# Gaurav14cs17/Bayer_Low_light_Image_Enhancement

Measured on AMD Instinct MI355X. Metric: megapixels/sec RawFormer-S 512x512 RAW->sRGB, higher is better.
Workload: dtype f32; 1 GPU; RawFormer-S(FLCA) dim=32, batch=8 of packed 4x512x512 synthetic Bayer per GPU; frames_per_gpu=8, variant=flca, weights=synthetic (seeded, random-init scale), parallelism=batch-sharded x1, device=AMD Radeon Graphics

## Files before the change

### bayer_low_light_image_enhancement_amd/csrc/rf_conv3x3.hip

```cpp
#include <cstdio>
#include <cstdlib>
#include "rf_common.h"

namespace rf {

static constexpr int KC = 8;
static constexpr int kKsCounters = 4096;
typedef unsigned u32x4 __attribute__((ext_vector_type(4)));

template <int NCO, int LOG2_RW, int RPW, int NWV, bool KS = false>
__global__ void __launch_bounds__(64 * NWV, (NWV >= 8 || NCO >= 3) ? 1 : 2) conv3x3_kernel(Conv3x3Args a, int ngroups, int tiles_x, int ntiles, int vec) {
    constexpr int NTHR = 64 * NWV;
    constexpr int TAPS = 18;
    constexpr int NM = 6;
    constexpr int RW = 1 << LOG2_RW;
    constexpr int TW = 64 / RW;
    constexpr int TH = NWV * RW * RPW;
    static_assert(RPW == 1 || RW == 1, "two row groups per wave only with one row per group");
    constexpr int RS = TW + 8;
    constexpr int PS = ((TH + 2) * RS + 63) / 64 * 64;
    constexpr int NIN = KC * (TH + 2) * (TW + 2);
    constexpr int EPT = (NIN + NTHR - 1) / NTHR;
    constexpr int NW4 = 2 * TAPS * NCO * 16;
    constexpr int WPT = (NW4 + NTHR - 1) / NTHR;
    constexpr int BUF = KC * PS + 2 * TAPS * NCO * 64;
    __shared__ __attribute__((aligned(16))) float lds[2 * BUF];
    __shared__ float bias_l[NCO * 16];

    const int tid = threadIdx.x;
    const int lane = tid & 63, wave = tid >> 6;
    const int j = lane & 15, kq = lane >> 4;
    const int rowj = j / (16 / RW), cg = j % (16 / RW);
    const int grp = blockIdx.x % ngroups;
    const int wg = blockIdx.x / ngroups;
    const int b = blockIdx.y;
    const int h = a.h, w = a.w;
    const int NT = (a.Cout + 15) >> 4;
    const int t0 = grp * NCO;
    const int nchunks_all = (a.Cin + KC - 1) / KC;
    const int ksplit = KS ? (int)gridDim.z : 1, kz = KS ? (int)blockIdx.z : 0;
    const int ch_lo = KS ? (int)((long)kz * nchunks_all / ksplit) : 0, ch_hi = KS ? (int)((long)(kz + 1) * nchunks_all / ksplit) : nchunks_all;
    const float* xb = a.x + (size_t)b * a.x_bstride;
    const size_t chunk_stride = a.unshuffle_in ? (size_t)(KC / 4) * 4 * h * w : (size_t)KC * h * w;

    constexpr unsigned OOB = 0x80000000u;
    int prc[EPT];
    short loff[EPT];
    static_assert(PS - (TH + 2) * RS >= 16, "plane padding holds the dummy slots");
    const int dummy = (tid & 7) * PS + (TH + 2) * RS + ((tid >> 3) & 15);
#pragma unroll
    for (int i = 0; i < EPT; ++i) {
        const int idx = tid + NTHR * i;
        const int c = idx % (TW + 2);
        const int r = (idx / (TW + 2)) % (TH + 2);
        const int cl = idx / ((TW + 2) * (TH + 2));
        prc[i] = idx < NIN ? (cl << 16) | (r << 8) | c : -1;
        loff[i] = (short)(idx < NIN ? cl * PS + r * RS + c : dummy);
    }
    unsigned wvoff[WPT];
#pragma unroll
    for (int i = 0; i < WPT; ++i) {
        const int idx = tid + NTHR * i;
        const int l4 = idx % 16;
        const int t = (idx / 16) % NCO;
        const int kt = idx / (16 * NCO);
        const bool ok = idx < NW4 && t0 + t < NT;
        wvoff[i] = ok ? (unsigned)(((kt * NT + t0 + t) * 64 + l4 * 4) * 4) : OOB;
    }
    const int w_chunk_bytes = 2 * TAPS * NT * 64 * 4;
    const size_t plane_bytes = (size_t)h * w * 4;

    unsigned voff[EPT];
    int x0 = 0, y0 = 0;
    auto plan_tile = [&](int tile) {
        const int tx = tile % tiles_x, ty = tile / tiles_x;
        x0 = tx * TW;
        y0 = ty * TH;
#pragma unroll
        for (int i = 0; i < EPT; ++i) {
            int e = prc[i];
            asm volatile("" : "+v"(e));
            const int cl = e >> 16;
            const int y = y0 - 1 + ((e >> 8) & 255), x = x0 - 1 + (e & 255);
            const bool ok = e >= 0 && (unsigned)y < (unsigned)h && (unsigned)x < (unsigned)w;
            const int off_m = ((cl >> 2) * 2 * h + 2 * y + ((cl >> 1) & 1)) * (2 * w) + 2 * x + (cl & 1);
            const int off_p = (cl * h + y) * w + x;
            voff[i] = ok ? (unsigned)(4 * (a.unshuffle_in ? off_m : off_p)) : OOB;
        }
    };
    float xin[EPT];
    float4 win[WPT];
    auto load_chunk = [&](int ch) {
        const int cl_lim = min(KC, a.Cin - ch * KC);
        const float* src = xb + (size_t)ch * chunk_stride;
        const __amdgpu_buffer_rsrc_t rx = __builtin_amdgcn_make_buffer_rsrc(
            const_cast<float*>(src), 0, (int)(a.unshuffle_in ? (size_t)(cl_lim / 4) * 4 * plane_bytes : (size_t)cl_lim * plane_bytes), 0x00020000);
        const __amdgpu_buffer_rsrc_t rw = __builtin_amdgcn_make_buffer_rsrc(
            const_cast<float*>(a.wp) + (size_t)ch * (w_chunk_bytes / 4), 0, w_chunk_bytes, 0x00020000);
#pragma unroll
        for (int i = 0; i < EPT; ++i) xin[i] = __uint_as_float(__builtin_amdgcn_raw_buffer_load_b32(rx, (int)voff[i], 0, 0));
#pragma unroll
        for (int i = 0; i < WPT; ++i) {
            const u32x4 v = __builtin_amdgcn_raw_buffer_load_b128(rw, (int)wvoff[i], 0, 0);
            win[i] = make_float4(__uint_as_float(v.x), __uint_as_float(v.y), __uint_as_float(v.z), __uint_as_float(v.w));
        }
    };
    auto store_chunk = [&](int buf) {
        float* li = lds + buf * BUF;
        float* lw = li + KC * PS;
#pragma unroll
        for (int i = 0; i < EPT; ++i) {
            float v = xin[i];
            if (a.clamp_in) v = fminf(fmaxf(v, 0.f), 1.f);
            li[loff[i]] = v;
        }
#pragma unroll
        for (int i = 0; i < WPT; ++i) {
            const int idx = tid + NTHR * i;
            if (idx < NW4) *reinterpret_cast<float4*>(lw + idx * 4) = win[i];
        }
    };

    f32x4 acc[RPW][NCO][NM];

    const int nwg = gridDim.x / ngroups;
    int tile = wg;
    const int tile_end = ntiles;
    if (tile >= tile_end) return;
    if (tid < NCO * 16) {
        const int co = 16 * t0 + tid;
        bias_l[tid] = (a.bias && co < a.Cout) ? a.bias[co] : 0.f;
    }
    plan_tile(tile);
    load_chunk(ch_lo);
    store_chunk(0);
    __syncthreads();
    int buf = 0;
    float* outb = a.out + (size_t)b * a.out_bstride;
    for (; tile < tile_end; tile += nwg) {
        const int ex0 = x0, ey0 = y0;
#pragma unroll
        for (int rr = 0; rr < RPW; ++rr)
#pragma unroll
            for (int t = 0; t < NCO; ++t)
#pragma unroll
                for (int g = 0; g < NM; ++g) acc[rr][t][g] = (f32x4){0.f, 0.f, 0.f, 0.f};
        for (int ch = ch_lo; ch < ch_hi; ++ch) {
            const bool last = ch + 1 == ch_hi;
            const bool more = !last || tile + nwg < tile_end;
            const int nch = last ? ch_lo : ch + 1;
            if (last && more) plan_tile(tile + nwg);
            if (more) load_chunk(nch);
            const float* lds_in = lds + buf * BUF;
            const float* lds_w = lds_in + KC * PS;
            const int nks = (a.Cin - ch * KC > 4) ? 2 : 1;
#pragma unroll
            for (int ks = 0; ks < 2; ++ks) {
                if (ks >= nks) break;
                const float* lp = lds_in + (ks * 4 + kq) * PS + (wave * RW * RPW + rowj) * RS + 4 * cg;
#pragma unroll
                for (int ir = 0; ir < RPW + 2; ++ir) {
                    const float4 lo = *reinterpret_cast<const float4*>(lp + ir * RS);
                    const float4 hi = *reinterpret_cast<const float4*>(lp + ir * RS + 4);
                    float d[NM];
                    {
                        const float p = fmaf(-4.f, lo.z, hi.x), q = fmaf(-4.f, lo.y, lo.w);
                        const float c2 = hi.x - lo.z, e2 = lo.w - lo.y;
                        d[0] = fmaf(4.f, lo.x, fmaf(-5.f, lo.z, hi.x));
                        d[1] = p + q; d[2] = p - q;
                        d[3] = fmaf(2.f, e2, c2); d[4] = fmaf(-2.f, e2, c2);
                        d[5] = fmaf(4.f, lo.y, fmaf(-5.f, lo.w, hi.y));
                    }
#pragma unroll
                    for (int rr = 0; rr < RPW; ++rr) {
                        const int dy = ir - rr;
                        if (dy < 0 || dy > 2) continue;
#pragma unroll
                        for (int j4 = 0; j4 < TAPS / 3; ++j4) {
                            const float* wl = lds_w + ((ks * TAPS + dy * (TAPS / 3) + j4) * NCO) * 64 + lane;
#pragma unroll
                            for (int t = 0; t < NCO; ++t) {
                                acc[rr][t][j4] = __builtin_amdgcn_mfma_f32_16x16x4f32(wl[t * 64], d[j4], acc[rr][t][j4], 0, 0, 0);
                            }
                        }
                    }
                }
            }
            if (more) store_chunk(buf ^ 1);
            __syncthreads();
            buf ^= 1;
        }

    int kq_ = kq;
    asm volatile("" : "+v"(kq_));
    const int x = ex0 + 4 * cg;
    auto transform = [&](int rr, int t, float (&u)[4][4]) {
        const f32x4* mm = acc[rr][t];
#pragma unroll
        for (int r = 0; r < 4; ++r) {
            const float s12 = mm[1][r] + mm[2][r], d12 = mm[1][r] - mm[2][r], s34 = mm[3][r] + mm[4][r], d34 = mm[3][r] - mm[4][r];
            u[r][0] = (mm[0][r] + s12) + s34;
            u[r][1] = fmaf(2.f, d34, d12);
            u[r][2] = fmaf(4.f, s34, s12);
            u[r][3] = fmaf(8.f, d34, d12) + mm[5][r];
        }
    };
    auto finish = [&](int t, float (&v)[4][4]) {
#pragma unroll
        for (int r = 0; r < 4; ++r) {
            const float bs = bias_l[16 * t + 4 * kq_ + r];
#pragma unroll
            for (int g = 0; g < 4; ++g) {
                float u = v[r][g] + bs;
                if (a.act == 1) u = u > 0.f ? u : 0.2f * u;
                else if (a.act == 2) u = fmaxf(u, 0.f);
                else if (a.act == 3) u = gelu_fast(u);
                else if (a.act == 4) u = 1.0f - 2.0f * __builtin_amdgcn_rcpf(1.0f + __expf(2.0f * u));
                if (a.clamp_out) u = fminf(fmaxf(u, 0.f), 1.f);
                v[r][g] = u;
            }
        }
    };
    auto store_tile = [&](int t, int y, const float (&v)[4][4]) {
        const int cobase = 16 * (t0 + t) + 4 * kq_;
        if (a.store == 0) {
#pragma unroll
            for (int r = 0; r < 4; ++r) {
                const int co = cobase + r;
                if (co >= a.Cout) continue;
                float* o = outb + ((size_t)co * h + y) * w + x;
                if (vec) {
                    *reinterpret_cast<float4*>(o) = make_float4(v[r][0], v[r][1], v[r][2], v[r][3]);
                } else {
#pragma unroll
                    for (int g = 0; g < 4; ++g)
                        if (x + g < w) o[g] = v[r][g];
                }
            }
        } else if (a.store == 1) {
            const int h2 = h >> 1, w2 = w >> 1;
#pragma unroll
            for (int r = 0; r < 4; ++r) {
                const int co = cobase + r;
                if (co >= a.Cout) continue;
                float* o = outb + (((size_t)(4 * co + 2 * (y & 1))) * h2 + (y >> 1)) * w2 + (x >> 1);
                const size_t ps = (size_t)h2 * w2;
                if (vec) {
                    *reinterpret_cast<float2*>(o) = make_float2(v[r][0], v[r][2]);
                    *reinterpret_cast<float2*>(o + ps) = make_float2(v[r][1], v[r][3]);
                } else {
#pragma unroll
                    for (int g = 0; g < 4; ++g)
                        if (x + g < w) o[(size_t)(g & 1) * ps + (g >> 1)] = v[r][g];
                }
            }
        } else {
            if (cobase >= a.Cout) return;
            const int c = cobase >> 2;
            float* op = outb + (size_t)c * 4 * h * w;
            const int w2 = 2 * w;
            if (vec) {
#pragma unroll
                for (int i = 0; i < 2; ++i) {
                    float* row = op + (size_t)(2 * y + i) * w2 + 2 * x;
                    *reinterpret_cast<float4*>(row) = make_float4(v[2 * i][0], v[2 * i + 1][0], v[2 * i][1], v[2 * i + 1][1]);
                    *reinterpret_cast<float4*>(row + 4) = make_float4(v[2 * i][2], v[2 * i + 1][2], v[2 * i][3], v[2 * i + 1][3]);
                }
            } else {
#pragma unroll
                for (int g = 0; g < 4; ++g)
                    if (x + g < w) {
#pragma unroll
                        for (int r = 0; r < 4; ++r)
                            op[(size_t)(2 * y + (r >> 1)) * w2 + 2 * (x + g) + (r & 1)] = v[r][g];
                    }
            }
        }
    };
    if constexpr (!KS) {
#pragma unroll
        for (int rr = 0; rr < RPW; ++rr) {
            const int y = ey0 + (wave * RPW + rr) * RW + rowj;
            if (y >= h || x >= w) continue;
#pragma unroll
            for (int t = 0; t < NCO; ++t) {
                if (t0 + t >= NT) break;
                float v[4][4];
                transform(rr, t, v);
                finish(t, v);
                store_tile(t, y, v);
            }
        }
    } else {
        unsigned* counter = reinterpret_cast<unsigned*>(a.ks_scratch) + ((size_t)b * ntiles + tile) * ngroups + grp;
        float* part = a.ks_scratch + kKsCounters;
        const size_t split_stride = (size_t)a.B * a.Cout * h * w;
        float* mine = part + (size_t)kz * split_stride + (size_t)b * a.Cout * h * w;
#pragma unroll
        for (int rr = 0; rr < RPW; ++rr) {
            const int y = ey0 + (wave * RPW + rr) * RW + rowj;
            if (y >= h || x >= w) continue;
#pragma unroll
            for (int t = 0; t < NCO; ++t) {
                if (t0 + t >= NT) break;
                float v[4][4];
                transform(rr, t, v);
#pragma unroll
                for (int r = 0; r < 4; ++r) {
                    const int co = 16 * (t0 + t) + 4 * kq_ + r;
                    if (co < a.Cout) *reinterpret_cast<float4*>(mine + ((size_t)co * h + y) * w + x) = make_float4(v[r][0], v[r][1], v[r][2], v[r][3]);
                }
            }
        }
        __shared__ unsigned ticket;
        __builtin_amdgcn_fence(__ATOMIC_RELEASE, "agent");
        __syncthreads();
        if (tid == 0) ticket = atomicAdd(counter, 1u);
        __syncthreads();
        if (ticket != (unsigned)(ksplit - 1)) return;
        if (tid == 0) *counter = 0u;
        __builtin_amdgcn_fence(__ATOMIC_ACQUIRE, "agent");
#pragma unroll
        for (int rr = 0; rr < RPW; ++rr) {
            const int y = ey0 + (wave * RPW + rr) * RW + rowj;
            if (y >= h || x >= w) continue;
#pragma unroll
            for (int t = 0; t < NCO; ++t) {
                if (t0 + t >= NT) break;
                float v[4][4];
#pragma unroll
                for (int r = 0; r < 4; ++r) {
                    const int co = 16 * (t0 + t) + 4 * kq_ + r;
                    float4 sum = make_float4(0.f, 0.f, 0.f, 0.f);
                    if (co < a.Cout) {
                        const float* src = part + (size_t)b * a.Cout * h * w + ((size_t)co * h + y) * w + x;
                        for (int z = 0; z < ksplit; ++z) {
                            const float4 pz = *reinterpret_cast<const float4*>(src + (size_t)z * split_stride);
                            sum.x += pz.x; sum.y += pz.y; sum.z += pz.z; sum.w += pz.w;
                        }
                    }
                    v[r][0] = sum.x; v[r][1] = sum.y; v[r][2] = sum.z; v[r][3] = sum.w;
                }
                finish(t, v);
                store_tile(t, y, v);
            }
        }
        return;
    }
    }
}

size_t conv3x3_ksplit_counter_bytes() { return (size_t)kKsCounters * sizeof(float); }
size_t conv3x3_ksplit_floats(int B, int Cout, int h, int w) {
    return ((long)B * h * w <= 16384) ? (size_t)kKsCounters + (size_t)8 * B * Cout * h * w : 0;
}

static int ksplit_for(const Conv3x3Args& a, int ntiles, int ngroups, int vec, const dim3& grid) {
    if (!a.ks_scratch || !vec || !aligned16(a.ks_scratch)) return 1;
    const long total = (long)ntiles * ngroups * a.B;
    const int nchunks = cdiv(a.Cin, KC);
    if (total > 64 || total > kKsCounters || nchunks < 8 || (long)grid.x != (long)ngroups * ntiles) return 1;
    int S = nchunks / 4;
    if (S > 8) S = 8;
    while (S > 1 && total * S > 256) --S;
    if (S < 2 || (size_t)kKsCounters + (size_t)S * a.B * a.Cout * a.h * a.w > a.ks_floats) return 1;
    return S;
}

template <int NCO>
static void launch_rw(const Conv3x3Args& a, int ngroups, int vec, bool small, hipStream_t st) {
    const int lrw = a.w > 32 ? 0 : (a.w > 16 ? 1 : 2);
    constexpr int RPWB = NCO <= 2 ? 2 : 1;
    auto grid_for_tiles = [&](int ntiles) {
        const long total = (long)ntiles * ngroups * a.B;
        const int wgs = cdiv(ntiles, (int)((total + 255) / 256));
        return dim3((unsigned)(ngroups * wgs), (unsigned)a.B);
    };
    if (small && lrw == 0) {
        const int txs = cdiv(a.w, 64), ntiles = txs * cdiv(a.h, 4);
        dim3 grid = grid_for_tiles(ntiles);
        const int S = ksplit_for(a, ntiles, ngroups, vec, grid);
        grid.z = (unsigned)S;
        if (S > 1) conv3x3_kernel<NCO, 0, 1, 4, true><<<grid, 256, 0, st>>>(a, ngroups, txs, ntiles, vec);
        else conv3x3_kernel<NCO, 0, 1, 4><<<grid, 256, 0, st>>>(a, ngroups, txs, ntiles, vec);
    } else if (NCO == 1 && lrw == 0 && a.h >= 16) {
        const int txs = cdiv(a.w, 64), ntiles = txs * cdiv(a.h, 16);
        conv3x3_kernel<1, 0, 1, 16><<<grid_for_tiles(ntiles), 1024, 0, st>>>(a, ngroups, txs, ntiles, vec);
    } else if (lrw == 0 && a.h >= 8 * RPWB) {
        const int txs = cdiv(a.w, 64), ntiles = txs * cdiv(a.h, 8 * RPWB);
        conv3x3_kernel<NCO, 0, RPWB, 8><<<grid_for_tiles(ntiles), 512, 0, st>>>(a, ngroups, txs, ntiles, vec);
    } else if (lrw == 0 && a.h >= 8) {
        const int txs = cdiv(a.w, 64), ntiles = txs * cdiv(a.h, 8);
        conv3x3_kernel<NCO, 0, 1, 8><<<grid_for_tiles(ntiles), 512, 0, st>>>(a, ngroups, txs, ntiles, vec);
    } else {
        const int txs = cdiv(a.w, 64 >> lrw), ntiles = txs * cdiv(a.h, 4 << lrw);
        dim3 grid = grid_for_tiles(ntiles);
        const int S = ksplit_for(a, ntiles, ngroups, vec, grid);
        grid.z = (unsigned)S;
        if (S > 1) {
            if (lrw == 0) conv3x3_kernel<NCO, 0, 1, 4, true><<<grid, 256, 0, st>>>(a, ngroups, txs, ntiles, vec);
            else if (lrw == 1) conv3x3_kernel<NCO, 1, 1, 4, true><<<grid, 256, 0, st>>>(a, ngroups, txs, ntiles, vec);
            else conv3x3_kernel<NCO, 2, 1, 4, true><<<grid, 256, 0, st>>>(a, ngroups, txs, ntiles, vec);
        } else if (lrw == 0) conv3x3_kernel<NCO, 0, 1, 4><<<grid, 256, 0, st>>>(a, ngroups, txs, ntiles, vec);
        else if (lrw == 1) conv3x3_kernel<NCO, 1, 1, 4><<<grid, 256, 0, st>>>(a, ngroups, txs, ntiles, vec);
        else conv3x3_kernel<NCO, 2, 1, 4><<<grid, 256, 0, st>>>(a, ngroups, txs, ntiles, vec);
    }
}

int launch_conv3x3(const Conv3x3Args& a, hipStream_t st) {
    RF_CHECK_ARG(a.B > 0 && a.B <= 65535 && a.Cin > 0 && a.Cout > 0 && a.h > 0 && a.w > 0, "conv3x3: bad sizes");
    RF_CHECK_ARG(a.store == 0 || (a.store == 1 && a.h % 2 == 0 && a.w % 2 == 0) || (a.store == 2 && a.Cout % 4 == 0),
                 "conv3x3: store mode %d incompatible with Cout=%d h=%d w=%d", a.store, a.Cout, a.h, a.w);
    RF_CHECK_ARG(!a.unshuffle_in || a.Cin == 4, "conv3x3: the packed-mosaic input path takes exactly 4 channels");
    RF_CHECK_ARG((double)a.Cin * a.h * a.w * 4.0 < 2.0e9, "conv3x3: image too large for 32-bit gather offsets");
    const int NT = cdiv(a.Cout, 16);
    int nco = 4;
    if (NT % 4 != 0) nco = (NT % 3 == 0) ? 3 : (NT % 2 == 0 ? 2 : (NT == 1 ? 1 : 4));
    bool small = false;
    if (a.w > 32 && a.h >= 8) {
        const long big = (long)cdiv(a.w, 64) * cdiv(a.h, nco <= 2 ? 16 : 8) * cdiv(NT, nco) * a.B;
        if (big < 128) {
            small = true;
            const long t4 = (long)cdiv(a.w, 64) * cdiv(a.h, 4) * a.B;
            while (nco > 1 && t4 * cdiv(NT, nco) < 192) nco = (nco == 4 || nco == 2) ? nco / 2 : 1;
        }
    }
    const int ngroups = cdiv(NT, nco);
    const int vec = (a.w % 4 == 0) && aligned16(a.out) && (a.out_bstride % 4 == 0);
    char key[64];
    {
        const int lrw = a.w > 32 ? 0 : (a.w > 16 ? 1 : 2), rpwb = nco <= 2 ? 2 : 1;
        const int wide = lrw == 0 && a.h >= 8;
        snprintf(key, sizeof(key), "conv3x3_kernel<%d, %d, %d, %d>", nco, lrw, (wide && a.h >= 8 * rpwb) ? rpwb : 1, wide ? 8 : 4);
        if (nco == 1 && lrw == 0 && a.h >= 16) snprintf(key, sizeof(key), "conv3x3_kernel<1, 0, 1, 16>");
        if (small) snprintf(key, sizeof(key), "conv3x3_kernel<%d, 0, 1, 4>", nco);
    }
    const double px = (double)a.B * a.h * a.w;
    ProfScope prof(st, key, 18.0 * a.Cin * a.Cout * px, 4.0 * px * (a.Cin + a.Cout));
    switch (nco) {
        case 4: launch_rw<4>(a, ngroups, vec, small, st); break;
        case 3: launch_rw<3>(a, ngroups, vec, small, st); break;
        case 2: launch_rw<2>(a, ngroups, vec, small, st); break;
        default: launch_rw<1>(a, ngroups, vec, small, st); break;
    }
    return check_launch("conv3x3");
}

}
```

Measured before the change: 1053 MP/s.

## Add level-0 conv3x3 path with resident LDS weights and vectorized row loads

Adds a specialized conv3x3 variant for full-resolution layers (Cin<=32, NCO<=2, wide tiles). All weight chunks are loaded into LDS once per block rather than being double-buffered per chunk, and input rows are fetched with 128-bit buffer loads plus one scalar halo element per thread instead of per-element 32-bit loads. The epilogue is also restructured to read the bias as a float4 and hoist the activation branch out of the element loop. This cuts global load instruction count and per-chunk weight traffic, at the cost of more LDS per block, which may lower occupancy.

```diff
diff --git a/bayer_low_light_image_enhancement_amd/csrc/rf_conv3x3.hip b/bayer_low_light_image_enhancement_amd/csrc/rf_conv3x3.hip
--- a/bayer_low_light_image_enhancement_amd/csrc/rf_conv3x3.hip
+++ b/bayer_low_light_image_enhancement_amd/csrc/rf_conv3x3.hip
@@ -8,7 +8,7 @@
 static constexpr int kKsCounters = 4096;
 typedef unsigned u32x4 __attribute__((ext_vector_type(4)));
 
-template <int NCO, int LOG2_RW, int RPW, int NWV, bool KS = false>
+template <int NCO, int LOG2_RW, int RPW, int NWV, bool KS = false, int L0 = 0>
 __global__ void __launch_bounds__(64 * NWV, (NWV >= 8 || NCO >= 3) ? 1 : 2) conv3x3_kernel(Conv3x3Args a, int ngroups, int tiles_x, int ntiles, int vec) {
     constexpr int NTHR = 64 * NWV;
     constexpr int TAPS = 18;
@@ -19,13 +19,20 @@
     static_assert(RPW == 1 || RW == 1, "two row groups per wave only with one row per group");
     constexpr int RS = TW + 8;
     constexpr int PS = ((TH + 2) * RS + 63) / 64 * 64;
+    constexpr bool RESW = (L0 & 1) != 0, ROWS = (L0 & 2) != 0;
+    static_assert(L0 == 0 || (!KS && LOG2_RW == 0), "the level-0 path: wide tiles, no input-channel split");
     constexpr int NIN = KC * (TH + 2) * (TW + 2);
-    constexpr int EPT = (NIN + NTHR - 1) / NTHR;
-    constexpr int NW4 = 2 * TAPS * NCO * 16;
-    constexpr int WPT = (NW4 + NTHR - 1) / NTHR;
-    constexpr int BUF = KC * PS + 2 * TAPS * NCO * 64;
-    __shared__ __attribute__((aligned(16))) float lds[2 * BUF];
-    __shared__ float bias_l[NCO * 16];
+    constexpr int NV4 = KC * (TH + 2) * (TW / 4);
+    constexpr int V4PT = ROWS ? (NV4 + NTHR - 1) / NTHR : 0;
+    static_assert(!ROWS || 2 * KC * (TH + 2) <= NTHR, "one halo element per thread");
+    constexpr int EPT = ROWS ? V4PT + 1 : (NIN + NTHR - 1) / NTHR;
+    constexpr int WSL = 2 * TAPS * NCO * 64;
+    constexpr int NW4 = WSL / 4;
+    constexpr int WPT = RESW ? 0 : (NW4 + NTHR - 1) / NTHR;
+    constexpr int BUF = KC * PS + (RESW ? 0 : WSL);
+    constexpr int MAXCH = 32 / KC;
+    __shared__ __attribute__((aligned(16))) float lds[2 * BUF + (RESW ? MAXCH * WSL : 0)];
+    __shared__ __attribute__((aligned(16))) float bias_l[NCO * 16];
 
     const int tid = threadIdx.x;
     const int lane = tid & 63, wave = tid >> 6;
@@ -46,18 +53,34 @@
     constexpr unsigned OOB = 0x80000000u;
     int prc[EPT];
     short loff[EPT];
-    static_assert(PS - (TH + 2) * RS >= 16, "plane padding holds the dummy slots");
-    const int dummy = (tid & 7) * PS + (TH + 2) * RS + ((tid >> 3) & 15);
-#pragma unroll
-    for (int i = 0; i < EPT; ++i) {
-        const int idx = tid + NTHR * i;
-        const int c = idx % (TW + 2);
-        const int r = (idx / (TW + 2)) % (TH + 2);
-        const int cl = idx / ((TW + 2) * (TH + 2));
-        prc[i] = idx < NIN ? (cl << 16) | (r << 8) | c : -1;
-        loff[i] = (short)(idx < NIN ? cl * PS + r * RS + c : dummy);
-    }
-    unsigned wvoff[WPT];
+    static_assert(PS - (TH + 2) * RS >= (ROWS ? 32 : 16), "plane padding holds the dummy slots");
+    const int dummy = ROWS ? (tid & 7) * PS + (TH + 2) * RS + 4 * ((tid >> 3) & 7)
+                           : (tid & 7) * PS + (TH + 2) * RS + ((tid >> 3) & 15);
+    if constexpr (ROWS) {
+#pragma unroll
+        for (int i = 0; i < V4PT; ++i) {
+            const int idx = tid + NTHR * i;
+            const int c = 1 + 4 * (idx % (TW / 4));
+            const int r = (idx / (TW / 4)) % (TH + 2);
+            const int cl = idx / ((TW / 4) * (TH + 2));
+            prc[i] = idx < NV4 ? (cl << 16) | (r << 8) | c : -1;
+            loff[i] = (short)(idx < NV4 ? cl * PS + r * RS + c : dummy);
+        }
+        const int c = (tid & 1) * (TW + 1), r = (tid >> 1) % (TH + 2), cl = (tid >> 1) / (TH + 2);
+        prc[V4PT] = cl < KC ? (cl << 16) | (r << 8) | c : -1;
+        loff[V4PT] = (short)(cl < KC ? cl * PS + r * RS + c : dummy);
+    } else {
+#pragma unroll
+        for (int i = 0; i < EPT; ++i) {
+            const int idx = tid + NTHR * i;
+            const int c = idx % (TW + 2);
+            const int r = (idx / (TW + 2)) % (TH + 2);
+            const int cl = idx / ((TW + 2) * (TH + 2));
+            prc[i] = idx < NIN ? (cl << 16) | (r << 8) | c : -1;
+            loff[i] = (short)(idx < NIN ? cl * PS + r * RS + c : dummy);
+        }
+    }
+    unsigned wvoff[WPT > 0 ? WPT : 1];
 #pragma unroll
     for (int i = 0; i < WPT; ++i) {
         const int idx = tid + NTHR * i;
@@ -88,8 +111,9 @@
             voff[i] = ok ? (unsigned)(4 * (a.unshuffle_in ? off_m : off_p)) : OOB;
         }
     };
-    float xin[EPT];
-    float4 win[WPT];
+    float xin[ROWS ? 1 : EPT];
+    u32x4 xin4[ROWS ? V4PT : 1];
+    float4 win[WPT > 0 ? WPT : 1];
     auto load_chunk = [&](int ch) {
         const int cl_lim = min(KC, a.Cin - ch * KC);
         const float* src = xb + (size_t)ch * chunk_stride;
@@ -97,8 +121,14 @@
             const_cast<float*>(src), 0, (int)(a.unshuffle_in ? (size_t)(cl_lim / 4) * 4 * plane_bytes : (size_t)cl_lim * plane_bytes), 0x00020000);
         const __amdgpu_buffer_rsrc_t rw = __builtin_amdgcn_make_buffer_rsrc(
             const_cast<float*>(a.wp) + (size_t)ch * (w_chunk_bytes / 4), 0, w_chunk_bytes, 0x00020000);
-#pragma unroll
-        for (int i = 0; i < EPT; ++i) xin[i] = __uint_as_float(__builtin_amdgcn_raw_buffer_load_b32(rx, (int)voff[i], 0, 0));
+        if constexpr (ROWS) {
+#pragma unroll
+            for (int i = 0; i < V4PT; ++i) xin4[i] = __builtin_amdgcn_raw_buffer_load_b128(rx, (int)voff[i], 0, 0);
+            xin[0] = __uint_as_float(__builtin_amdgcn_raw_buffer_load_b32(rx, (int)voff[V4PT], 0, 0));
+        } else {
+#pragma unroll
+            for (int i = 0; i < EPT; ++i) xin[i] = __uint_as_float(__builtin_amdgcn_raw_buffer_load_b32(rx, (int)voff[i], 0, 0));
+        }
 #pragma unroll
         for (int i = 0; i < WPT; ++i) {
             const u32x4 v = __builtin_amdgcn_raw_buffer_load_b128(rw, (int)wvoff[i], 0, 0);
@@ -108,11 +138,22 @@
     auto store_chunk = [&](int buf) {
         float* li = lds + buf * BUF;
         float* lw = li + KC * PS;
-#pragma unroll
-        for (int i = 0; i < EPT; ++i) {
+        if constexpr (ROWS) {
+#pragma unroll
+            for (int i = 0; i < V4PT; ++i) {
+#pragma unroll
+                for (int g = 0; g < 4; ++g) {
+                    float v = __uint_as_float(xin4[i][g]);
+                    if (a.clamp_in) v = fminf(fmaxf(v, 0.f), 1.f);
+                    li[loff[i] + g] = v;
+                }
+            }
+        }
+#pragma unroll
+        for (int i = 0; i < (ROWS ? 1 : EPT); ++i) {
             float v = xin[i];
             if (a.clamp_in) v = fminf(fmaxf(v, 0.f), 1.f);
-            li[loff[i]] = v;
+            li[loff[ROWS ? V4PT : i]] = v;
         }
 #pragma unroll
         for (int i = 0; i < WPT; ++i) {
@@ -133,6 +174,16 @@
     }
     plan_tile(tile);
     load_chunk(ch_lo);
+    if constexpr (RESW) {
+        float* lw = lds + 2 * BUF;
+        const int n4 = nchunks_all * NW4;
+        for (int idx = tid; idx < n4; idx += NTHR) {
+            const int l4 = idx % 16, t = (idx / 16) % NCO, kt = idx / (16 * NCO);
+            float4 v = make_float4(0.f, 0.f, 0.f, 0.f);
+            if (t0 + t < NT) v = *reinterpret_cast<const float4*>(a.wp + ((size_t)(kt * NT + t0 + t) * 64 + l4 * 4));
+            *reinterpret_cast<float4*>(lw + idx * 4) = v;
+        }
+    }
     store_chunk(0);
     __syncthreads();
     int buf = 0;
@@ -152,7 +203,7 @@
             if (last && more) plan_tile(tile + nwg);
             if (more) load_chunk(nch);
             const float* lds_in = lds + buf * BUF;
-            const float* lds_w = lds_in + KC * PS;
+            const float* lds_w = RESW ? lds + 2 * BUF + ch * WSL : lds_in + KC * PS;
             const int nks = (a.Cin - ch * KC > 4) ? 2 : 1;
 #pragma unroll
             for (int ks = 0; ks < 2; ++ks) {
@@ -206,19 +257,24 @@
         }
     };
     auto finish = [&](int t, float (&v)[4][4]) {
-#pragma unroll
-        for (int r = 0; r < 4; ++r) {
-            const float bs = bias_l[16 * t + 4 * kq_ + r];
-#pragma unroll
-            for (int g = 0; g < 4; ++g) {
-                float u = v[r][g] + bs;
-                if (a.act == 1) u = u > 0.f ? u : 0.2f * u;
-                else if (a.act == 2) u = fmaxf(u, 0.f);
-                else if (a.act == 3) u = gelu_fast(u);
-                else if (a.act == 4) u = 1.0f - 2.0f * __builtin_amdgcn_rcpf(1.0f + __expf(2.0f * u));
-                if (a.clamp_out) u = fminf(fmaxf(u, 0.f), 1.f);
-                v[r][g] = u;
-            }
+        const float4 b4 = *reinterpret_cast<const float4*>(bias_l + 16 * t + 4 * kq_);
+        const float bs[4] = {b4.x, b4.y, b4.z, b4.w};
+        auto each = [&](auto f) {
+#pragma unroll
+            for (int r = 0; r < 4; ++r)
+#pragma unroll
+                for (int g = 0; g < 4; ++g) v[r][g] = f(v[r][g] + bs[r]);
+        };
+        if (a.act == 1) each([](float u) { return u > 0.f ? u : 0.2f * u; });
+        else if (a.act == 2) each([](float u) { return fmaxf(u, 0.f); });
+        else if (a.act == 3) each([](float u) { return gelu_fast(u); });
+        else if (a.act == 4) each([](float u) { return 1.0f - 2.0f * __builtin_amdgcn_rcpf(1.0f + __expf(2.0f * u)); });
+        else each([](float u) { return u; });
+        if (a.clamp_out) {
+#pragma unroll
+            for (int r = 0; r < 4; ++r)
+#pragma unroll
+                for (int g = 0; g < 4; ++g) v[r][g] = fminf(fmaxf(v[r][g], 0.f), 1.f);
         }
     };
     auto store_tile = [&](int t, int y, const float (&v)[4][4]) {
@@ -367,6 +423,11 @@
     return S;
 }
 
+static bool level0_path(const Conv3x3Args& a, int nco, bool small) {
+    return !small && nco <= 2 && a.w > 32 && a.h >= 16 && a.Cin <= 32 && !a.unshuffle_in && a.w % 4 == 0 && aligned16(a.x) &&
+           a.x_bstride % 4 == 0;
+}
+
 template <int NCO>
 static void launch_rw(const Conv3x3Args& a, int ngroups, int vec, bool small, hipStream_t st) {
     const int lrw = a.w > 32 ? 0 : (a.w > 16 ? 1 : 2);
@@ -385,9 +446,16 @@
         else conv3x3_kernel<NCO, 0, 1, 4><<<grid, 256, 0, st>>>(a, ngroups, txs, ntiles, vec);
     } else if (NCO == 1 && lrw == 0 && a.h >= 16) {
         const int txs = cdiv(a.w, 64), ntiles = txs * cdiv(a.h, 16);
-        conv3x3_kernel<1, 0, 1, 16><<<grid_for_tiles(ntiles), 1024, 0, st>>>(a, ngroups, txs, ntiles, vec);
+        if (level0_path(a, NCO, small)) conv3x3_kernel<1, 0, 1, 16, false, 3><<<grid_for_tiles(ntiles), 1024, 0, st>>>(a, ngroups, txs, ntiles, vec);
+        else conv3x3_kernel<1, 0, 1, 16><<<grid_for_tiles(ntiles), 1024, 0, st>>>(a, ngroups, txs, ntiles, vec);
     } else if (lrw == 0 && a.h >= 8 * RPWB) {
         const int txs = cdiv(a.w, 64), ntiles = txs * cdiv(a.h, 8 * RPWB);
+        if constexpr (NCO == 2) {
+            if (level0_path(a, NCO, small)) {
+                conv3x3_kernel<2, 0, 2, 8, false, 3><<<grid_for_tiles(ntiles), 512, 0, st>>>(a, ngroups, txs, ntiles, vec);
+                return;
+            }
+        }
         conv3x3_kernel<NCO, 0, RPWB, 8><<<grid_for_tiles(ntiles), 512, 0, st>>>(a, ngroups, txs, ntiles, vec);
     } else if (lrw == 0 && a.h >= 8) {
         const int txs = cdiv(a.w, 64), ntiles = txs * cdiv(a.h, 8);
@@ -434,6 +502,7 @@
         snprintf(key, sizeof(key), "conv3x3_kernel<%d, %d, %d, %d>", nco, lrw, (wide && a.h >= 8 * rpwb) ? rpwb : 1, wide ? 8 : 4);
         if (nco == 1 && lrw == 0 && a.h >= 16) snprintf(key, sizeof(key), "conv3x3_kernel<1, 0, 1, 16>");
         if (small) snprintf(key, sizeof(key), "conv3x3_kernel<%d, 0, 1, 4>", nco);
+        if (level0_path(a, nco, small)) snprintf(key, sizeof(key), "conv3x3_kernel<%d, 0, %d, %d, false, 3>", nco, nco == 1 ? 1 : 2, nco == 1 ? 16 : 8);
     }
     const double px = (double)a.B * a.h * a.w;
     ProfScope prof(st, key, 18.0 * a.Cin * a.Cout * px, 4.0 * px * (a.Cin + a.Cout));
```

Result: faster. 1083 MP/s, median of 6 (+2.8%).
